# facebookresearch/theseus

Hardware: AMD Instinct MI355X
Metric: LM iterations/sec (batch x vars) on SE3 pose-graph (higher is better)
Workload: dtype f32

## Files before the change

include/theseus_hip.h:

```cpp
#ifndef THESEUS_HIP_H_
#define THESEUS_HIP_H_

#include <stdint.h>

#ifdef __cplusplus
extern "C" {
#endif

#define THX_F32 0
#define THX_F64 1
#define THX_TILE 128

typedef struct {
  double near_zero;
  double d_near_zero;
  double near_pi;
} thx_lie_eps;

typedef struct {
  int32_t num_poses;
  int32_t num_edges;
  int32_t num_priors;
  const int32_t* edge_i;
  const int32_t* edge_j;
// ... 121 lines not shown
  const int32_t* th_mask32;
  const int32_t* th_k0h;
  const int32_t* rg0_rows;
  const int32_t* rg0_zf;
  const int32_t* rg0_tile_ptr;
  const int32_t* rg0_piece_blk;
  const int32_t* rg0_piece_rc;
  int32_t rg0_ngroups;
  int32_t rg0_max_tile_pieces;
  const int32_t* sc_pair_host;
  const int32_t* sc_perm;
  const int32_t* sc_mask;
  const int32_t* row_first;
} thx_hblock_layout;
int thx_hblock_fill_mask(int32_t nvars, int32_t bd, int32_t nblocks, const int32_t* blocks, int32_t* mask);
int thx_pg_assemble_blocks(const thx_pg_structure* s, const thx_pg_data* d, const thx_hblock_layout* layout, void* Hc,
                           int64_t bstride, void* g, int dtype, const thx_lie_eps* eps, void* stream);
int thx_hblocks_expand(const thx_hblock_layout* layout, const void* Hc, int64_t bstride, int32_t B, void* H, int64_t ld,
                       int dtype, void* stream);
int thx_hblocks_diag(const thx_hblock_layout* layout, const void* Hc, int64_t bstride, int32_t B, void* d, int64_t ldv,
                     int dtype, void* stream);

typedef struct {
  int32_t row0, col0, dof_a, dof_b, term_begin, term_end, elem_begin, pad_;
} thx_block_target;
typedef struct {
  const void* Ja;
  const void* Jb;
  int64_t bstride_a, bstride_b;
  int32_t dim, dof_a, dof_b, pad_;
// ... 309 lines not shown
```

theseus_amd/_lib.py:

```python
import ctypes
import os
from ctypes import POINTER, Structure, c_char_p, c_double, c_int, c_int32, c_int64, c_void_p

import torch

_HERE = os.path.dirname(os.path.abspath(__file__))
LIB_PATH = os.environ.get("THESEUS_HIP_LIB") or os.path.join(_HERE, "lib", "libtheseus_hip.so")

THX_TILE = 128
THX_ERR_CHUNKS = 128
THX_LU_MAX_N = 4096
THX_BA_ERR_CHUNKS = 256
TRAJ2_COLLISION, TRAJ2_GP, TRAJ2_PRIOR = 0, 1, 2
PUSH2_QSP, PUSH2_MFB, PUSH2_CONTACT, PUSH2_PRIOR = 0, 1, 2, 3
HOMOG_ALIGN, HOMOG_PRIOR = 0, 1
THX_HOMOG_CHUNK = 1024
THX_HOMOG_SUMS = 10
LOSS_NONE, LOSS_WELSCH, LOSS_HUBER, LOSS_HINGE = 0, 1, 2, 3
LOSS_FLATTEN = 4
LOSS_GEMAN_MCCLURE = 8
ABI_VERSION = 30


class LieEps(Structure):
# ... 59 lines not shown
        (k, c_void_p) for k in ("rg_group_ptr_host", "rg_rows", "rg_k0", "rg_tile_ptr", "rg_piece_blk", "rg_piece_rc")] + [
        ("rg_max_tile_pieces", c_int32)] + [
        (k, c_void_p) for k in ("rg_zf", "tr_tile_host", "tr_perm16", "tr_mask16", "th_tile_host", "th_perm32", "th_mask32", "th_k0h",
                                "rg0_rows", "rg0_zf", "rg0_tile_ptr", "rg0_piece_blk", "rg0_piece_rc")] + [
        ("rg0_ngroups", c_int32), ("rg0_max_tile_pieces", c_int32)] + [
        (k, c_void_p) for k in ("sc_pair_host", "sc_perm", "sc_mask", "row_first")]


def hblock_fill_mask(blocks, nvars: int, bd: int):
    import numpy as np
    b = np.ascontiguousarray(np.asarray(blocks, dtype=np.int32).reshape(-1, 2))
    ntiles = (nvars * bd + THX_TILE - 1) // THX_TILE
    mask = np.zeros((ntiles, 4 * ntiles), dtype=np.int32)
    check(load().thx_hblock_fill_mask(nvars, bd, b.shape[0], b.ctypes.data, mask.ctypes.data), "thx_hblock_fill_mask")
    return mask


def max_offdiag_tile_pieces(tile_ptr, ntiles: int) -> int:
    import numpy as np
    cnt = np.diff(np.asarray(tile_ptr, dtype=np.int64))
    if cnt.size < ntiles * (ntiles + 1) // 2 or ntiles < 2:
        return 0
    off = np.ones(ntiles * (ntiles + 1) // 2, bool)
    i = np.arange(ntiles)
    off[i * (i + 1) // 2 + i] = False
    return int(cnt[: off.size][off].max())


class SE2Eps(Structure):
    _fields_ = [("near_zero", c_double), ("d_near_zero", c_double)]
# ... 92 lines not shown
                        c_void_p, c_int, c_void_p, POINTER(CholSchedule)],
    "thx_chol_factor_forward": [c_void_p, c_int64, c_int32, c_int32, c_void_p, c_int, c_double, c_void_p, c_void_p,
                                c_void_p, c_void_p, c_void_p, c_int64, c_int, c_void_p, POINTER(CholSchedule)],
    "thx_chol_factor_sparse": [c_void_p, c_int64, c_int32, c_int32, c_void_p, c_int, c_double, c_void_p, c_void_p, c_void_p,
                               c_void_p, c_void_p, c_int64, POINTER(TilePattern), c_int, c_void_p, POINTER(CholSchedule)],
    "thx_chol_solve_sparse": [c_void_p, c_int64, c_int32, c_int32, c_void_p, c_void_p, c_void_p, c_int64, c_int,
                              POINTER(TilePattern), c_int, c_void_p],
    "thx_pg_assemble_blocks": [POINTER(PGStructure), POINTER(PGData), POINTER(HBlockLayout), c_void_p, c_int64, c_void_p, c_int,
                               POINTER(LieEps), c_void_p],
    "thx_hblocks_expand": [POINTER(HBlockLayout), c_void_p, c_int64, c_int32, c_void_p, c_int64, c_int, c_void_p],
    "thx_hblocks_diag": [POINTER(HBlockLayout), c_void_p, c_int64, c_int32, c_void_p, c_int64, c_int, c_void_p],
    "thx_chol_factor_hblocks": [POINTER(HBlockLayout), c_void_p, c_int64, c_int32, c_int32, c_void_p, c_int, c_double, c_void_p,
                                c_int64, c_void_p, c_void_p, c_void_p, c_void_p, c_int64, POINTER(TilePattern), c_int, c_void_p,
                                POINTER(CholSchedule)],
    "thx_hblock_fill_mask": [c_int32, c_int32, c_int32, c_void_p, c_void_p],
    "thx_chol_plan": [c_int32, c_int64, c_int32, c_int, c_int, c_int, c_int64, POINTER(HBlockLayout), POINTER(CholSchedule),
                      POINTER(CholPlanInfo)],
    "thx_chol_factor_levels": [POINTER(HBlockLayout), c_void_p, c_int64, c_int32, c_void_p, c_int, c_double, c_void_p, c_void_p,
                               c_void_p, c_void_p, c_void_p, c_int64, POINTER(TilePattern), POINTER(LevelSchedule), c_int, c_void_p,
                               POINTER(CholSchedule)],
    "thx_chol_solve_levels": [c_void_p, c_int32, c_void_p, c_void_p, c_void_p, c_int64, c_int, POINTER(TilePattern),
                              POINTER(LevelSchedule), c_int, c_void_p],
    "thx_vec_gather": [c_void_p, c_int64, c_void_p, c_int64, c_void_p, c_int32, c_int32, c_int, c_void_p],
    "thx_chol_solve": [c_void_p, c_int64, c_int32, c_int32, c_void_p, c_void_p, c_void_p, c_int64, c_int,
                       c_void_p],
    "thx_chol_solve_backward": [c_void_p, c_int64, c_int32, c_int32, c_void_p, c_void_p, c_void_p, c_int64, c_int,
                                c_void_p],
    "thx_chol_solve_env": [c_void_p, c_int64, c_int32, c_int32, c_void_p, c_void_p, c_void_p, c_int64, c_void_p, c_int,
                           c_void_p],
    "thx_chol_solve_backward_env": [c_void_p, c_int64, c_int32, c_int32, c_void_p, c_void_p, c_void_p, c_int64, c_void_p, c_int,
# ... 96 lines not shown
```

theseus_amd/build.py:

```python
import os
import re
import subprocess
import sys

HERE = os.path.dirname(os.path.abspath(__file__))
CSRC = os.path.join(HERE, "csrc")
LIBDIR = os.path.join(HERE, "lib")
LIB = os.path.join(LIBDIR, "libtheseus_hip.so")
SOURCES = ["pg_kernels.hip", "chol_kernels.hip", "pg_vjp_kernels.hip", "block_kernels.hip", "pg2_kernels.hip", "ba_kernels.hip", "pgso3_kernels.hip", "pgso2_kernels.hip", "ba_vjp_kernels.hip", "vjp_unroll_ba_kernels.hip", "lu_kernels.hip", "multi_solve_kernels.hip", "traj_kernels.hip", "push_kernels.hip", "homog_kernels.hip"]
FLAGS = ["--offload-arch=gfx950", "-O3", "-std=c++17", "-fPIC", "-Wno-unused-value", "-Wno-pass-failed"]


def _mtime(p):
    return os.path.getmtime(p) if os.path.exists(p) else 0.0


def deps(path):
    seen, todo = set(), [os.path.normpath(path)]
    while todo:
        f = todo.pop()
        if f in seen:
            continue
        seen.add(f)
        with open(f) as fh:
# ... 30 lines not shown
```

theseus_amd/compiler.py:

```python
from dataclasses import dataclass, field
from typing import List, Optional, Sequence, Tuple

import numpy as np
import torch

from . import _lib

DOF = 6


@dataclass
class PoseGraphStructure:

    num_poses: int
    edge_i: np.ndarray
    edge_j: np.ndarray
    prior_pose: np.ndarray
    edge_row_start: np.ndarray = None
    prior_row_start: np.ndarray = None
    inc_ptr: np.ndarray = field(default=None, repr=False)
    inc_edge: np.ndarray = field(default=None, repr=False)
    inc_side: np.ndarray = field(default=None, repr=False)
    inc_other: np.ndarray = field(default=None, repr=False)
    pri_ptr: np.ndarray = field(default=None, repr=False)
# ... 520 lines not shown
                self.t["sc_" + f] = torch.from_numpy(np.ascontiguousarray(getattr(pc, f))).to(device)
                setattr(c, "sc_" + f, self.t["sc_" + f].data_ptr())
        tr = hb.tile_rows()
        if tr is not None:
            self.tr_tile_host = np.ascontiguousarray(tr.has)
            c.tr_tile_host = self.tr_tile_host.ctypes.data
            for f in ("perm", "mask"):
                self.t["tr_" + f + "16"] = torch.from_numpy(np.ascontiguousarray(getattr(tr, f))).to(device)
                setattr(c, "tr_" + f + "16", self.t["tr_" + f + "16"].data_ptr())
            self.th_tile_host = np.ascontiguousarray(tr.has32)
            c.th_tile_host = self.th_tile_host.ctypes.data
            for f in ("perm32", "mask32", "k0h"):
                self.t["th_" + f] = torch.from_numpy(np.ascontiguousarray(getattr(tr, f))).to(device)
                setattr(c, "th_" + f, self.t["th_" + f].data_ptr())
        self.c = c
```

theseus_amd/kernels.py:

```python
import ctypes
import dataclasses
from dataclasses import dataclass
from typing import Callable, Optional

import torch

from . import _lib
from .compiler import DeviceStructure

_LIE_EPS = {
    torch.float32: dict(near_zero=1e-2, d_near_zero=2e-1, near_pi=1e-2),
    torch.float64: dict(near_zero=5e-3, d_near_zero=1e-2, near_pi=1e-7),
}
_SE2_EPS = {
    torch.float32: dict(near_zero=3e-2, d_near_zero=1e-1),
    torch.float64: dict(near_zero=1e-6, d_near_zero=1e-3),
}
_FLAGS = dict(fast_approx_local_jacobians=False)
_REFERENCE_PARAMS = None


def use_reference_global_params(theseus_params) -> None:
    global _REFERENCE_PARAMS
    _REFERENCE_PARAMS = theseus_params
# ... 375 lines not shown
    def pg_assemble_blocks(self, s: DeviceStructure, t: PGTensors, hb, Hc, g, poses=None):
        if t.group != "SE3":
            raise RuntimeError("the block-compact Hessian is implemented for SE3 pose graphs")
        dt = Hc.dtype
        _lib.check(self.lib.thx_pg_assemble_blocks(s.c, t.c_struct(poses), hb.c, _lib.ptr(Hc, "Hc"), Hc.stride(0), _lib.ptr(g, "g"),
                                                   _lib.dtype_code(dt), lie_eps(dt), _lib.stream_ptr(Hc.device)),
                   "thx_pg_assemble_blocks")

    def hblocks_expand(self, hb, Hc, H):
        _lib.check(self.lib.thx_hblocks_expand(hb.c, _lib.ptr(Hc), Hc.stride(0), Hc.shape[0], _lib.ptr(H), H.shape[-1],
                                               _lib.dtype_code(Hc.dtype), _lib.stream_ptr(Hc.device)), "thx_hblocks_expand")

    def hblocks_diag(self, hb, Hc, d):
        _lib.check(self.lib.thx_hblocks_diag(hb.c, _lib.ptr(Hc), Hc.stride(0), Hc.shape[0], _lib.ptr(d), d.stride(0),
                                             _lib.dtype_code(Hc.dtype), _lib.stream_ptr(Hc.device)), "thx_hblocks_diag")

    def chol_factor_hblocks(self, hb, Hc, n, damping, ellipsoidal, damping_eps, L, panels, info, pattern=None, rhs=None, y=None):
        B, ld = L.shape[0], (0 if L.dim() == 4 else L.shape[-1])
        _lib.check(self.lib.thx_chol_factor_hblocks(
            hb.c, _lib.ptr(Hc), Hc.stride(0), n, B, _lib.ptr(damping), int(bool(ellipsoidal)), float(damping_eps), _lib.ptr(L), ld,
            _lib.ptr(panels), _lib.ptr(info), _lib.ptr(rhs), _lib.ptr(y), rhs.stride(0) if rhs is not None else n,
            pattern.c_struct(L.device) if pattern is not None else None, _lib.dtype_code(L.dtype), _lib.stream_ptr(L.device),
            self._sched()), "thx_chol_factor_hblocks")

    def chol_factor_levels(self, layout, Hc, damping, ellipsoidal, damping_eps, L, panels, info, pattern, rhs=None, y=None):
        dev = L.device
        _lib.check(self.lib.thx_chol_factor_levels(
            layout.c, _lib.ptr(Hc), Hc.stride(0), L.shape[0], _lib.ptr(damping), int(bool(ellipsoidal)), float(damping_eps),
            _lib.ptr(L), _lib.ptr(panels), _lib.ptr(info), _lib.ptr(rhs), _lib.ptr(y), y.stride(0) if y is not None else 0,
            pattern.c_struct(dev), pattern.c_levels(dev), _lib.dtype_code(L.dtype), _lib.stream_ptr(dev), self._sched()),
# ... 410 lines not shown
```

theseus_amd/linear_solver.py:

```python
import abc
import math
import warnings
from typing import Any, Dict, Optional, Sequence, Type, Union

import torch

from .core import Objective
from .linearization import HipLinearization, Linearization
from . import _lib


class LinearSolver(abc.ABC):
    def __init__(self, objective: Objective, linearization_cls: Optional[Type[Linearization]] = None,
                 linearization_kwargs: Optional[Dict[str, Any]] = None, **kwargs):
        linearization_kwargs = linearization_kwargs or {}
        self.linearization: Linearization = linearization_cls(objective, **linearization_kwargs)

    def reset(self, **kwargs):
        pass

    @abc.abstractmethod
    def solve(self, damping: Optional[Union[float, torch.Tensor]] = None, **kwargs) -> torch.Tensor:
        pass


class HipCholeskyCore:

    def _core_init(self):
        self.K = self.linearization.K
        self.L = self.panels = self.info = self._y = None
        self._lam = None
        self.factor_version = 0

    def _ensure_buffers(self):
        lin = self.linearization
        g = lin.g
        shape = (g.shape[0], lin.ld, lin.ld)
        if self.L is None or tuple(self.L.shape) != shape or self.L.device != g.device or self.L.dtype != g.dtype:
            B = g.shape[0]
            nt = (lin.n + _lib.THX_TILE - 1) // _lib.THX_TILE
            self.L = torch.zeros(shape, dtype=g.dtype, device=g.device)
            self.panels = torch.empty(B, nt, _lib.THX_TILE, _lib.THX_TILE, dtype=g.dtype, device=g.device)
            self._y = torch.empty(B, lin.n, dtype=g.dtype, device=g.device)
            self.info = torch.zeros(B, dtype=torch.int32, device=g.device)
            self._lam = torch.empty(B, dtype=g.dtype, device=g.device)
            self._unfused_forward = False

    def _linearized(self) -> bool:
        lin = self.linearization
        return lin.linearized if hasattr(lin, "linearized") else lin.H is not None

    def _factor_call(self, lam, ellipsoidal_damping, damping_eps, rhs, y, pattern=None):
        lin = self.linearization
        if getattr(lin, "_compact", False):
            self.K.chol_factor_hblocks(lin.hblocks, lin.Hc, lin.n, lam, ellipsoidal_damping, damping_eps, self.L, self.panels,
                                       self.info, pattern=pattern, rhs=rhs, y=y)
        elif pattern is not None:
            self.K.chol_factor_sparse(lin.H, lin.n, lam, ellipsoidal_damping, damping_eps, self.L, self.panels, self.info,
                                      pattern, rhs=rhs, y=y)
        else:
            self.K.chol_factor(lin.H, lin.n, lam, ellipsoidal_damping, damping_eps, self.L, self.panels, self.info, rhs=rhs, y=y)

    def factorize(self, damping: Optional[Union[float, torch.Tensor]] = None, ellipsoidal_damping: bool = True,
                  damping_eps: float = 1e-8, rhs: Optional[torch.Tensor] = None):
        if not self._linearized():
            raise RuntimeError("linearize() must be called before solve().")
        self._ensure_buffers()
        lam = None
        if damping is not None:
            lam = self._lam
            if isinstance(damping, torch.Tensor):
                lam.copy_(damping.to(lam.dtype).expand(lam.shape[0]))
            else:
                lam.fill_(float(damping))
        y = self._y if rhs is not None else None
        self.factor_version += 1
        self._factored_with = (lam is not None, bool(ellipsoidal_damping), float(damping_eps))
        self._factor_call(lam, ellipsoidal_damping, damping_eps, rhs, y)
        return y

    def solve_with_factor(self, rhs: torch.Tensor) -> torch.Tensor:
        rhs = rhs.contiguous()
        x = torch.empty_like(rhs)
        self._substitute(rhs, x, backward_only=False)
        return x

    def factor_snapshot(self):
        return self.L.clone(), self.panels.clone()

    def solve_with_snapshot(self, snapshot, rhs: torch.Tensor) -> torch.Tensor:
        L, panels = snapshot
        rhs = rhs.contiguous()
        x = torch.empty_like(rhs)
        self.K.chol_solve(L, self.linearization.n, panels, rhs, x, **self._envelope())
        return x

    solve_envelope = True

    def _envelope(self) -> Dict[str, torch.Tensor]:
        lin = self.linearization
        if self.solve_envelope and getattr(lin, "_compact", False) and lin.hblocks is not None:
            return {"row_first": lin.hblocks.t["row_first"]}
        return {}

    def _substitute(self, rhs, x, backward_only: bool):
        if backward_only:
            self.K.chol_solve_backward(self.L, self.linearization.n, self.panels, rhs, x, **self._envelope())
        else:
            self.K.chol_solve(self.L, self.linearization.n, self.panels, rhs, x, **self._envelope())

    def _factor_owner(self) -> "HipCholeskyCore":
        return self

    def _factorize_undamped(self) -> "HipCholeskyCore":
        self.factorize(None)
        self.check_info()
        return self

    def solve_multi_with_factor(self, rhs: torch.Tensor, which: int = 0) -> torch.Tensor:
        own = self._factor_owner()
        if own is None or own.L is None or own.factor_version == 0:
            raise RuntimeError("solve_multi_with_factor: nothing has been factorised yet (solve() or factorize() first).")
        n = own.linearization.n
        if rhs.dim() != 3 or rhs.shape[0] != own.L.shape[0] or rhs.shape[2] != n or rhs.shape[1] < 1:
            raise ValueError(f"solve_multi_with_factor: rhs must be (B = {own.L.shape[0]}, k >= 1, n = {n}), got {tuple(rhs.shape)}")
        x = rhs.detach().to(own.L.dtype).clone(memory_format=torch.contiguous_format)
        own.K.chol_solve_multi(own.L, n, own.panels, x, x, which=which)
        return x

    @torch.no_grad()
    def sample_deltas(self, n_samples: int = 10, temperature: float = 1.0, noise: Optional[torch.Tensor] = None,
                      generator: Optional[torch.Generator] = None) -> torch.Tensor:
        if not temperature > 0:
            raise ValueError(f"sample_deltas: temperature must be positive, got {temperature}")
        if int(n_samples) < 1:
            raise ValueError(f"sample_deltas: n_samples must be at least 1, got {n_samples}")
        delta = self.solve()
        own = self._factor_owner()
        B, n = delta.shape
        if noise is None:
            noise = torch.randn(n, int(n_samples), generator=generator, device=delta.device, dtype=delta.dtype)
        if noise.dim() == 2 and tuple(noise.shape) == (n, n_samples):
            y = noise.t().unsqueeze(0).expand(B, n_samples, n)
        elif noise.dim() == 3 and tuple(noise.shape) == (B, n, n_samples):
            y = noise.transpose(1, 2)
        else:
            raise ValueError(f"sample_deltas: noise must be ({n}, {n_samples}) or ({B}, {n}, {n_samples}), got {tuple(noise.shape)}")
        y = y.to(device=delta.device, dtype=delta.dtype).clone(memory_format=torch.contiguous_format)
        own.K.chol_solve_multi(own.L, n, own.panels, y, y, which=1)
        y.mul_(math.sqrt(float(temperature))).add_(delta.unsqueeze(1))
        return y.transpose(1, 2)

    @torch.no_grad()
    def marginal_covariance(self, var_names: Sequence[str]) -> torch.Tensor:
        lin = self.linearization
        names = list(var_names)
        if len(set(names)) != len(names):
            raise ValueError(f"marginal_covariance: repeated variable names in {names}")
        cols = []
        for name in names:
            try:
                k = lin.ordering.index_of(name)
            except KeyError:
                raise ValueError(f"marginal_covariance: {name!r} is not an optimisation variable of the objective") from None
            cols.extend(range(lin.var_start_cols[k], lin.var_start_cols[k] + lin.var_dims[k]))
        if not cols:
            raise ValueError("marginal_covariance: no variables named")
        own = self._factorize_undamped()
        B, n, d = own.L.shape[0], own.linearization.n, len(cols)
        idx = torch.tensor(cols, dtype=torch.long, device=own.L.device)
        E = torch.zeros(B, d, n, dtype=own.L.dtype, device=own.L.device)
        E[:, torch.arange(d, device=idx.device), idx] = 1
        own.K.chol_solve_multi(own.L, n, own.panels, E, E, which=0)
        C = E[:, :, idx]
        return (C + C.transpose(1, 2)) / 2

    def check_info(self):
        bad = self.info.nonzero()
        if bad.numel():
            b = int(bad[0])
            raise RuntimeError(
                f"linalg.cholesky: (Batch element {b}): The factorization could not be completed because the "
                f"input is not positive-definite (the leading minor of order {int(self.info[b])} is not "
                "positive-definite).")

    def singular_mask(self) -> torch.Tensor:
        return (self.linearization.diagonal() == 0).any(dim=1)

# ... 28 lines not shown
            singular = self.singular_mask()
            self._last_singular = singular
            delta.masked_fill_(singular.unsqueeze(1), 0.0)
            self.info.masked_fill_(singular, 0)
            seen = singular.any()
            self._singular_seen = seen if getattr(self, "_singular_seen", None) is None else (self._singular_seen | seen)
            if check_info:
                self.post_singular_warning()
        if check_info:
            self.check_info()
        return delta


class HipCholeskySolver(HipCholeskyCore, LinearSolver):
    def __init__(self, objective: Objective, linearization_cls: Optional[Type[Linearization]] = None,
                 linearization_kwargs: Optional[Dict[str, Any]] = None, check_singular: bool = False, **kwargs):
        linearization_cls = linearization_cls or HipLinearization
        if not (isinstance(linearization_cls, type) and issubclass(linearization_cls, HipLinearization)):
            raise RuntimeError("HipCholeskySolver only works with theseus_amd.HipLinearization, "
                               f"but {linearization_cls} was provided.")
        LinearSolver.__init__(self, objective, linearization_cls, linearization_kwargs)
        self._check_singular = check_singular
        self._core_init()

    def solve(self, damping: Optional[Union[float, torch.Tensor]] = None, ellipsoidal_damping: bool = True,
              damping_eps: float = 1e-8, check_info: bool = True, **kwargs) -> torch.Tensor:
        return self._solve(damping, ellipsoidal_damping, damping_eps, check_info)


def _dense_cholesky_only(name: str):
    def method(self, *args, **kwargs):
# ... 62 lines not shown
    def _substitute(self, rhs, x, backward_only: bool):
        if backward_only:
            self.K.lu_solve_backward(self.LU, self.linearization.n, rhs, x)
        else:
            self.K.lu_solve(self.LU, self.linearization.n, self.piv, rhs, x)

    def check_info(self):
        bad = self.info.nonzero()
        if bad.numel():
            b = int(bad[0])
            raise RuntimeError(f"linalg.solve: (Batch element {b}): The solver failed because the input matrix is singular.")


class HipLUSolver(HipLUCore, LinearSolver):
    def __init__(self, objective: Objective, linearization_cls: Optional[Type[Linearization]] = None,
                 linearization_kwargs: Optional[Dict[str, Any]] = None, check_singular: bool = False, **kwargs):
        linearization_cls = linearization_cls or HipLinearization
        if not (isinstance(linearization_cls, type) and issubclass(linearization_cls, HipLinearization)):
            raise RuntimeError("HipLUSolver only works with theseus_amd.HipLinearization, "
                               f"but {linearization_cls} was provided.")
        LinearSolver.__init__(self, objective, linearization_cls, linearization_kwargs)
        self._check_singular = check_singular
        self._core_init()

    def solve(self, damping: Optional[Union[float, torch.Tensor]] = None, ellipsoidal_damping: bool = True,
              damping_eps: float = 1e-8, check_info: bool = True, **kwargs) -> torch.Tensor:
        return self._solve(damping, ellipsoidal_damping, damping_eps, check_info)
```

theseus_amd/plugin.py:

```python
from typing import Any, Dict, List, Optional, Type, Union

import torch

import theseus as th
from theseus.optimizer import Linearization as _RefLinearization
from theseus.optimizer.linear import CholeskyDenseSolver as _RefCholeskyDenseSolver
from theseus.optimizer.linear import LUDenseSolver as _RefLUDenseSolver
from theseus.optimizer.linear import LinearSolver as _RefLinearSolver

from theseus.global_params import _THESEUS_GLOBAL_PARAMS as _REF_GLOBAL_PARAMS

from .generic import BlockAssembler
from .autograd import detached_tensors, pg_vjp_grads
from .kernels import default_kernels, round_up
from .linear_solver import HipCholeskyCore, HipLUCore
from .linearization import HipLinearizationCore
from .packed import UnsupportedObjective
from . import kernels as _kernels

_kernels.use_reference_global_params(_REF_GLOBAL_PARAMS)


def _refuse_unrolled_av(lin):
    if getattr(lin, "_unroll", None) is not None and torch.is_grad_enabled():
# ... 470 lines not shown
        self.K.diag(self.H, self.n, d)
        return d


class _TensorSystemSolver(HipCholeskyCore):
    def __init__(self, K, check_singular: bool):
        self.linearization = _TensorSystem(K)
        self._check_singular = check_singular
        self._core_init()


class HipCholeskySolver(HipCholeskyCore, _RefCholeskyDenseSolver):

    def __init__(self, objective: th.Objective, linearization_cls: Optional[Type[_RefLinearization]] = None,
                 linearization_kwargs: Optional[Dict[str, Any]] = None, check_singular: bool = False,
                 lagged_failure_check: bool = False, **kwargs):
        linearization_cls = linearization_cls or HipLinearization
        if not (isinstance(linearization_cls, type) and issubclass(linearization_cls, HipLinearization)):
            raise RuntimeError("HipCholeskySolver only works with theseus_amd.plugin.HipLinearization, "
                               f"but {linearization_cls} was provided.")
        _RefLinearSolver.__init__(self, objective, linearization_cls, linearization_kwargs)
        self._check_singular = check_singular
        self._core_init()
        self._lagged = bool(lagged_failure_check)
        self._lag = None

    def reset(self, **kwargs):
        if self._lagged and self._lag is not None and self._lag.seen():
            self._lag = None
            import warnings
            warnings.warn("HipCholeskySolver(lagged_failure_check=True): the last linear solve of the previous optimize() failed "
# ... 303 lines not shown
```

Before: 107,900.

## Add fill-reducing variable reordering for sparse Cholesky of compact Hessian blocks

Adds a host-side reordering pass (Cuthill-McKee and King orderings scored by envelope size) that permutes pose variables to shrink the envelope of the block Hessian. The compact Hessian blocks are permuted on device into the new order, factored there, and the right-hand side and solution are gathered into and out of the permuted frame. It aims to cut the fill and work of the envelope/tiled Cholesky factor and solve. It adds permute and gather kernels each iteration plus a one-time ordering cost, and it is only used when the ordering beats the natural order.

Result: faster. 131,200 (median of 6 runs) (+21.6%).

```diff
diff --git a/include/theseus_hip.h b/include/theseus_hip.h
--- a/include/theseus_hip.h
+++ b/include/theseus_hip.h
@@ -159,6 +159,11 @@
   const int32_t* row_first;
 } thx_hblock_layout;
 int thx_hblock_fill_mask(int32_t nvars, int32_t bd, int32_t nblocks, const int32_t* blocks, int32_t* mask);
+int thx_hblock_order(int32_t nvars, int32_t bd, int32_t nblocks, const int32_t* blocks, int32_t* perm_out, int64_t* score_out);
+int thx_hblocks_permute(const void* src, int64_t sstride, void* dst, int64_t dstride, const int32_t* map, int32_t nblocks, int32_t bd,
+                        int32_t B, int dtype, void* stream);
+int thx_frame_permute(const void* H, int64_t ld, void* Hp, int64_t ldp, const int32_t* idx, int32_t n, int32_t B, int dtype,
+                      void* stream);
 int thx_pg_assemble_blocks(const thx_pg_structure* s, const thx_pg_data* d, const thx_hblock_layout* layout, void* Hc,
                            int64_t bstride, void* g, int dtype, const thx_lie_eps* eps, void* stream);
 int thx_hblocks_expand(const thx_hblock_layout* layout, const void* Hc, int64_t bstride, int32_t B, void* H, int64_t ld,
diff --git a/theseus_amd/_lib.py b/theseus_amd/_lib.py
--- a/theseus_amd/_lib.py
+++ b/theseus_amd/_lib.py
@@ -97,6 +97,15 @@
     mask = np.zeros((ntiles, 4 * ntiles), dtype=np.int32)
     check(load().thx_hblock_fill_mask(nvars, bd, b.shape[0], b.ctypes.data, mask.ctypes.data), "thx_hblock_fill_mask")
     return mask
+
+
+def hblock_order(blocks, nvars: int, bd: int):
+    import numpy as np
+    b = np.ascontiguousarray(np.asarray(blocks, dtype=np.int32).reshape(-1, 2))
+    perm = np.zeros(nvars, dtype=np.int32)
+    score = np.zeros(2, dtype=np.int64)
+    check(load().thx_hblock_order(nvars, bd, b.shape[0], b.ctypes.data, perm.ctypes.data, score.ctypes.data), "thx_hblock_order")
+    return perm, int(score[0]), int(score[1])
 
 
 def max_offdiag_tile_pieces(tile_ptr, ntiles: int) -> int:
@@ -219,6 +228,9 @@
                                 c_int64, c_void_p, c_void_p, c_void_p, c_void_p, c_int64, POINTER(TilePattern), c_int, c_void_p,
                                 POINTER(CholSchedule)],
     "thx_hblock_fill_mask": [c_int32, c_int32, c_int32, c_void_p, c_void_p],
+    "thx_hblock_order": [c_int32, c_int32, c_int32, c_void_p, c_void_p, c_void_p],
+    "thx_hblocks_permute": [c_void_p, c_int64, c_void_p, c_int64, c_void_p, c_int32, c_int32, c_int32, c_int, c_void_p],
+    "thx_frame_permute": [c_void_p, c_int64, c_void_p, c_int64, c_void_p, c_int32, c_int32, c_int, c_void_p],
     "thx_chol_plan": [c_int32, c_int64, c_int32, c_int, c_int, c_int, c_int64, POINTER(HBlockLayout), POINTER(CholSchedule),
                       POINTER(CholPlanInfo)],
     "thx_chol_factor_levels": [POINTER(HBlockLayout), c_void_p, c_int64, c_int32, c_void_p, c_int, c_double, c_void_p, c_void_p,
diff --git a/theseus_amd/build.py b/theseus_amd/build.py
--- a/theseus_amd/build.py
+++ b/theseus_amd/build.py
@@ -7,7 +7,7 @@
 CSRC = os.path.join(HERE, "csrc")
 LIBDIR = os.path.join(HERE, "lib")
 LIB = os.path.join(LIBDIR, "libtheseus_hip.so")
-SOURCES = ["pg_kernels.hip", "chol_kernels.hip", "pg_vjp_kernels.hip", "block_kernels.hip", "pg2_kernels.hip", "ba_kernels.hip", "pgso3_kernels.hip", "pgso2_kernels.hip", "ba_vjp_kernels.hip", "vjp_unroll_ba_kernels.hip", "lu_kernels.hip", "multi_solve_kernels.hip", "traj_kernels.hip", "push_kernels.hip", "homog_kernels.hip"]
+SOURCES = ["pg_kernels.hip", "chol_kernels.hip", "hblock_order.hip", "pg_vjp_kernels.hip", "block_kernels.hip", "pg2_kernels.hip", "ba_kernels.hip", "pgso3_kernels.hip", "pgso2_kernels.hip", "ba_vjp_kernels.hip", "vjp_unroll_ba_kernels.hip", "lu_kernels.hip", "multi_solve_kernels.hip", "traj_kernels.hip", "push_kernels.hip", "homog_kernels.hip"]
 FLAGS = ["--offload-arch=gfx950", "-O3", "-std=c++17", "-fPIC", "-Wno-unused-value", "-Wno-pass-failed"]
 
 
diff --git a/theseus_amd/compiler.py b/theseus_amd/compiler.py
--- a/theseus_amd/compiler.py
+++ b/theseus_amd/compiler.py
@@ -558,3 +558,53 @@
                 self.t["th_" + f] = torch.from_numpy(np.ascontiguousarray(getattr(tr, f))).to(device)
                 setattr(c, "th_" + f, self.t["th_" + f].data_ptr())
         self.c = c
+
+
+class _OrderedPattern:
+
+    def __init__(self, dof: int, nvars: int, pattern: np.ndarray):
+        self.dof, self.num_poses, self._pattern = dof, nvars, pattern
+        self.inc_ptr = np.zeros(nvars + 1, dtype=np.int32)
+        self.inc_other = np.zeros(0, dtype=np.int32)
+
+    def lower_block_pattern(self) -> np.ndarray:
+        return self._pattern
+
+
+class OrderedHessianBlocks:
+
+    def __init__(self, hb: HessianBlocks, perm: np.ndarray):
+        d, P = hb.bd, hb.nvars
+        perm = np.asarray(perm, dtype=np.int64)
+        if perm.shape != (P,) or not np.array_equal(np.sort(perm), np.arange(P)):
+            raise ValueError("OrderedHessianBlocks: perm is not a permutation of the layout's variables")
+        pos = np.empty(P, dtype=np.int64)
+        pos[perm] = np.arange(P)
+        a, b = pos[hb.blocks[:, 0]], pos[hb.blocks[:, 1]]
+        swapped = a < b
+        pat = np.stack([np.maximum(a, b), np.minimum(a, b)], axis=1)
+        self.base, self.perm, self.pos = hb, perm.astype(np.int32), pos.astype(np.int32)
+        self.layout = HessianBlocks(_OrderedPattern(d, P, pat[np.lexsort((pat[:, 1], pat[:, 0]))]))
+        ident = {(int(p), int(q)): k for k, (p, q) in enumerate(self.layout.blocks.tolist())}
+        self.block_map = np.zeros(hb.nblocks, dtype=np.int32)
+        for k, ((p, q), t) in enumerate(zip(pat.tolist(), swapped.tolist())):
+            self.block_map[ident[(p, q)]] = (k << 1) | int(t)
+        self.nswapped = int(swapped.sum())
+        self.to_perm = (d * perm[:, None] + np.arange(d)[None, :]).reshape(-1).astype(np.int32)
+        self.from_perm = (d * pos[:, None] + np.arange(d)[None, :]).reshape(-1).astype(np.int32)
+        self._dev = {}
+
+    def on(self, device):
+        key = str(device)
+        if key not in self._dev:
+            maps = {f: torch.from_numpy(getattr(self, f)).to(device) for f in ("block_map", "to_perm", "from_perm")}
+            self._dev[key] = (self.layout.on(device), maps)
+        return self._dev[key]
+
+
+def ordered_hessian_blocks(hb: HessianBlocks) -> Optional[OrderedHessianBlocks]:
+    cached = getattr(hb, "_ordered", None)
+    if cached is None:
+        perm, score, natural = _lib.hblock_order(hb.blocks, hb.nvars, hb.bd)
+        cached = hb._ordered = OrderedHessianBlocks(hb, perm) if score < natural else False
+    return cached or None
diff --git a/theseus_amd/csrc/hblock_order.hip b/theseus_amd/csrc/hblock_order.hip
--- /dev/null
+++ b/theseus_amd/csrc/hblock_order.hip
@@ -0,0 +1,280 @@
+#include <algorithm>
+#include <cstdint>
+#include <vector>
+
+#include "common.cuh"
+
+namespace thx {
+namespace {
+
+struct VarGraph {
+  int32_t n = 0;
+  std::vector<int32_t> ptr, adj;
+  int32_t deg(int32_t v) const { return ptr[v + 1] - ptr[v]; }
+};
+
+bool build_graph(int32_t nvars, int32_t nblocks, const int32_t* blocks, VarGraph& g) {
+  std::vector<std::pair<int32_t, int32_t>> e;
+  e.reserve(2 * (size_t)nblocks);
+  for (int32_t k = 0; k < nblocks; ++k) {
+    const int32_t p = blocks[2 * k], q = blocks[2 * k + 1];
+    if (p < 0 || p >= nvars || q < 0 || q > p) return false;
+    if (q < p) {
+      e.emplace_back(p, q);
+      e.emplace_back(q, p);
+    }
+  }
+  std::sort(e.begin(), e.end());
+  e.erase(std::unique(e.begin(), e.end()), e.end());
+  g.n = nvars;
+  g.ptr.assign(nvars + 1, 0);
+  g.adj.resize(e.size());
+  for (auto& x : e) ++g.ptr[x.first + 1];
+  for (int32_t v = 0; v < nvars; ++v) g.ptr[v + 1] += g.ptr[v];
+  for (size_t k = 0; k < e.size(); ++k) g.adj[k] = e[k].second;
+  return true;
+}
+
+int64_t envelope_score(const VarGraph& g, int32_t bd, const std::vector<int32_t>& order, std::vector<int32_t>& pos) {
+  for (int32_t k = 0; k < g.n; ++k) pos[order[k]] = k;
+  int64_t s = 0;
+  for (int32_t k = 0; k < g.n; ++k) {
+    const int32_t v = order[k];
+    int32_t f = k;
+    for (int32_t a = g.ptr[v]; a < g.ptr[v + 1]; ++a) f = std::min(f, pos[g.adj[a]]);
+    const int64_t w = (int64_t)bd * (k - f);
+    for (int32_t i = 0; i < bd; ++i) s += (w + i) * (w + i);
+  }
+  return s;
+}
+
+std::pair<int32_t, int32_t> bfs_far(const VarGraph& g, int32_t s, std::vector<int32_t>& level, std::vector<int32_t>& queue) {
+  std::fill(level.begin(), level.end(), -1);
+  queue.clear();
+  queue.push_back(s);
+  level[s] = 0;
+  for (size_t h = 0; h < queue.size(); ++h) {
+    const int32_t v = queue[h];
+    for (int32_t a = g.ptr[v]; a < g.ptr[v + 1]; ++a)
+      if (level[g.adj[a]] < 0) {
+        level[g.adj[a]] = level[v] + 1;
+        queue.push_back(g.adj[a]);
+      }
+  }
+  const int32_t last = level[queue.back()];
+  int32_t best = queue.back();
+  for (int32_t v : queue)
+    if (level[v] == last && (g.deg(v) < g.deg(best) || (g.deg(v) == g.deg(best) && v < best))) best = v;
+  return {best, last + 1};
+}
+
+std::pair<int32_t, int32_t> pseudo_peripheral(const VarGraph& g, int32_t s, std::vector<int32_t>& level, std::vector<int32_t>& queue) {
+  int32_t u = s;
+  auto fu = bfs_far(g, u, level, queue);
+  for (int it = 0; it < 8; ++it) {
+    const int32_t v = fu.first;
+    const auto fv = bfs_far(g, v, level, queue);
+    if (fv.second <= fu.second) return {u, v};
+    u = v;
+    fu = fv;
+  }
+  return {u, fu.first};
+}
+
+void cuthill_mckee(const VarGraph& g, int32_t start, std::vector<int32_t>& order) {
+  std::vector<char> seen(g.n, 0);
+  std::vector<int32_t> nb;
+  order.clear();
+  int32_t next_free = 0;
+  for (int32_t s = start; (int32_t)order.size() < g.n;) {
+    size_t h = order.size();
+    order.push_back(s);
+    seen[s] = 1;
+    for (; h < order.size(); ++h) {
+      const int32_t v = order[h];
+      nb.clear();
+      for (int32_t a = g.ptr[v]; a < g.ptr[v + 1]; ++a)
+        if (!seen[g.adj[a]]) nb.push_back(g.adj[a]);
+      std::sort(nb.begin(), nb.end(), [&](int32_t x, int32_t y) { return g.deg(x) != g.deg(y) ? g.deg(x) < g.deg(y) : x < y; });
+      for (int32_t w : nb) {
+        seen[w] = 1;
+        order.push_back(w);
+      }
+    }
+    while (next_free < g.n && seen[next_free]) ++next_free;
+    s = next_free;
+  }
+}
+
+void king(const VarGraph& g, int32_t start, std::vector<int32_t>& order) {
+  constexpr int32_t NUMBERED = -2, OUT = -1;
+  std::vector<int32_t> since(g.n, OUT);
+  std::vector<int32_t> front;
+  order.clear();
+  int32_t pick = start;
+  for (int32_t step = 0; step < g.n; ++step) {
+    if (pick < 0) {
+      int64_t bestg = INT64_MAX;
+      for (int32_t v : front) {
+        int32_t grow = 0;
+        for (int32_t a = g.ptr[v]; a < g.ptr[v + 1]; ++a) grow += since[g.adj[a]] == OUT;
+        const int64_t key = ((int64_t)grow << 32) | since[v];
+        if (key < bestg || (key == bestg && v < pick)) {
+          bestg = key;
+          pick = v;
+        }
+      }
+      if (pick < 0)
+        for (int32_t v = 0; v < g.n; ++v)
+          if (since[v] == OUT && (pick < 0 || g.deg(v) < g.deg(pick))) pick = v;
+    }
+    if (since[pick] >= 0) front.erase(std::find(front.begin(), front.end(), pick));
+    since[pick] = NUMBERED;
+    order.push_back(pick);
+    for (int32_t a = g.ptr[pick]; a < g.ptr[pick + 1]; ++a)
+      if (since[g.adj[a]] == OUT) {
+        since[g.adj[a]] = step;
+        front.push_back(g.adj[a]);
+      }
+    pick = -1;
+  }
+}
+
+}
+
+template <typename T>
+__global__ void hblocks_permute_kernel(const T* __restrict__ src, int64_t sstride, T* __restrict__ dst, int64_t dstride,
+                                       const int32_t* __restrict__ map, int nelems, int bd) {
+  const int b = blockIdx.y, idx = blockIdx.x * blockDim.x + threadIdx.x;
+  if (idx >= nelems) return;
+  const int bb = bd * bd, k = idx / bb, e = idx % bb;
+  const int m = map[k];
+  const int se = (m & 1) ? (e % bd) * bd + e / bd : e;
+  dst[(int64_t)b * dstride + idx] = src[(int64_t)b * sstride + (int64_t)(m >> 1) * bb + se];
+}
+
+template <typename T>
+__global__ void hblocks_permute4_kernel(const T* __restrict__ src, int64_t sstride, T* __restrict__ dst, int64_t dstride,
+                                        const int32_t* __restrict__ map, int nquads, int bd) {
+  typedef T T4 __attribute__((ext_vector_type(4)));
+  const int b = blockIdx.y, q = blockIdx.x * blockDim.x + threadIdx.x;
+  if (q >= nquads) return;
+  const int bb = bd * bd, qb = bb / 4, k = q / qb, e0 = 4 * (q % qb);
+  const int m = map[k];
+  const T* from = src + (int64_t)b * sstride + (int64_t)(m >> 1) * bb;
+  T4 v;
+  if (m & 1) {
+#pragma unroll
+    for (int i = 0; i < 4; ++i) v[i] = from[((e0 + i) % bd) * bd + (e0 + i) / bd];
+  } else {
+    v = *reinterpret_cast<const T4*>(from + e0);
+  }
+  *reinterpret_cast<T4*>(dst + (int64_t)b * dstride + (int64_t)k * bb + e0) = v;
+}
+
+template <typename T>
+__global__ void frame_permute_kernel(const T* __restrict__ H, int64_t ld, T* __restrict__ Hp, int64_t ldp,
+                                     const int32_t* __restrict__ idx, int n) {
+  const int b = blockIdx.z, i = blockIdx.y, j = blockIdx.x * blockDim.x + threadIdx.x;
+  if (j > i) return;
+  const int a = idx[i], c = idx[j];
+  Hp[(int64_t)b * ldp * ldp + (int64_t)i * ldp + j] = H[(int64_t)b * ld * ld + (int64_t)max(a, c) * ld + min(a, c)];
+}
+
+}
+
+using namespace thx;
+
+int thx_hblock_order(int32_t nvars, int32_t bd, int32_t nblocks, const int32_t* blocks, int32_t* perm_out, int64_t* score_out) {
+  if (nvars <= 0 || bd <= 0 || nblocks < 0 || (nblocks > 0 && !blocks) || !perm_out) return fail("thx_hblock_order: bad arguments");
+  if ((int64_t)nvars * bd > (int64_t)1 << 20) return fail("thx_hblock_order: matrix too large");
+  VarGraph g;
+  if (!build_graph(nvars, nblocks, blocks, g)) return fail("thx_hblock_order: a block outside tril(H)");
+  std::vector<int32_t> best(nvars), cand, rev, pos(nvars), level(nvars), queue;
+  for (int32_t v = 0; v < nvars; ++v) best[v] = v;
+  const int64_t natural = envelope_score(g, bd, best, pos);
+  int64_t best_score = natural;
+  auto offer = [&](const std::vector<int32_t>& o) {
+    const int64_t s = envelope_score(g, bd, o, pos);
+    if (s < best_score) {
+      best_score = s;
+      best = o;
+    }
+  };
+  auto offer_both = [&](const std::vector<int32_t>& o) {
+    offer(o);
+    rev.assign(o.rbegin(), o.rend());
+    offer(rev);
+  };
+  std::vector<int32_t> starts;
+  const auto ends = pseudo_peripheral(g, 0, level, queue);
+  starts = {ends.first, ends.second, 0, nvars - 1};
+  {
+    std::vector<int32_t> by_deg(nvars);
+    for (int32_t v = 0; v < nvars; ++v) by_deg[v] = v;
+    const int32_t take = std::min<int32_t>(4, nvars);
+    std::partial_sort(by_deg.begin(), by_deg.begin() + take, by_deg.end(),
+                      [&](int32_t x, int32_t y) { return g.deg(x) != g.deg(y) ? g.deg(x) < g.deg(y) : x < y; });
+    starts.insert(starts.end(), by_deg.begin(), by_deg.begin() + take);
+  }
+  {
+    std::vector<int32_t> uniq;
+    for (int32_t s : starts)
+      if (std::find(uniq.begin(), uniq.end(), s) == uniq.end()) uniq.push_back(s);
+    starts.swap(uniq);
+  }
+  cuthill_mckee(g, ends.first, cand);
+  offer_both(cand);
+  cuthill_mckee(g, ends.second, cand);
+  offer_both(cand);
+  if (nvars <= 16384)
+    for (int32_t s : starts) {
+      king(g, s, cand);
+      offer_both(cand);
+    }
+  std::copy(best.begin(), best.end(), perm_out);
+  if (score_out) {
+    score_out[0] = best_score;
+    score_out[1] = natural;
+  }
+  return 0;
+}
+
+int thx_hblocks_permute(const void* src, int64_t sstride, void* dst, int64_t dstride, const int32_t* map, int32_t nblocks, int32_t bd,
+                        int32_t B, int dtype, void* stream) {
+  if (!src || !dst || !map || nblocks <= 0 || bd <= 0 || B <= 0 || B > 65535 || src == dst) return fail("thx_hblocks_permute: bad args");
+  const int64_t nelems = (int64_t)nblocks * bd * bd;
+  if (nelems > INT32_MAX || sstride < nelems || dstride < nelems) return fail("thx_hblocks_permute: the lists are shorter than nblocks blocks");
+  const size_t vec = dtype == THX_F64 ? 32 : 16;
+  if ((bd * bd) % 4 == 0 && sstride % 4 == 0 && dstride % 4 == 0 && reinterpret_cast<uintptr_t>(src) % vec == 0 &&
+      reinterpret_cast<uintptr_t>(dst) % vec == 0) {
+    const int nquads = (int)(nelems / 4);
+    dim3 grid4((unsigned)((nquads + 255) / 256), B);
+    THX_DISPATCH(dtype,
+                 hipLaunchKernelGGL(hblocks_permute4_kernel<float>, grid4, dim3(256), 0, as_stream(stream), (const float*)src, sstride,
+                                    (float*)dst, dstride, map, nquads, bd),
+                 hipLaunchKernelGGL(hblocks_permute4_kernel<double>, grid4, dim3(256), 0, as_stream(stream), (const double*)src,
+                                    sstride, (double*)dst, dstride, map, nquads, bd));
+    return check_launch("thx_hblocks_permute");
+  }
+  dim3 grid((unsigned)((nelems + 255) / 256), B), block(256);
+  THX_DISPATCH(dtype,
+               hipLaunchKernelGGL(hblocks_permute_kernel<float>, grid, block, 0, as_stream(stream), (const float*)src, sstride,
+                                  (float*)dst, dstride, map, (int)nelems, bd),
+               hipLaunchKernelGGL(hblocks_permute_kernel<double>, grid, block, 0, as_stream(stream), (const double*)src, sstride,
+                                  (double*)dst, dstride, map, (int)nelems, bd));
+  return check_launch("thx_hblocks_permute");
+}
+
+int thx_frame_permute(const void* H, int64_t ld, void* Hp, int64_t ldp, const int32_t* idx, int32_t n, int32_t B, int dtype,
+                      void* stream) {
+  if (!H || !Hp || !idx || n <= 0 || n > 65535 || B <= 0 || B > 65535 || ld < n || ldp < n || H == Hp)
+    return fail("thx_frame_permute: bad args");
+  dim3 grid((n + 255) / 256, n, B), block(256);
+  THX_DISPATCH(dtype,
+               hipLaunchKernelGGL(frame_permute_kernel<float>, grid, block, 0, as_stream(stream), (const float*)H, ld, (float*)Hp,
+                                  ldp, idx, n),
+               hipLaunchKernelGGL(frame_permute_kernel<double>, grid, block, 0, as_stream(stream), (const double*)H, ld,
+                                  (double*)Hp, ldp, idx, n));
+  return check_launch("thx_frame_permute");
+}
diff --git a/theseus_amd/kernels.py b/theseus_amd/kernels.py
--- a/theseus_amd/kernels.py
+++ b/theseus_amd/kernels.py
@@ -413,6 +413,20 @@
     def hblocks_diag(self, hb, Hc, d):
         _lib.check(self.lib.thx_hblocks_diag(hb.c, _lib.ptr(Hc), Hc.stride(0), Hc.shape[0], _lib.ptr(d), d.stride(0),
                                              _lib.dtype_code(Hc.dtype), _lib.stream_ptr(Hc.device)), "thx_hblocks_diag")
+
+    def hblocks_permute(self, src, dst, block_map, bd):
+        if src.dim() != 2 or dst.dim() != 2 or src.shape[0] != dst.shape[0] or src.dtype != dst.dtype or block_map.dtype != torch.int32:
+            raise ValueError(f"hblocks_permute: src {tuple(src.shape)} {src.dtype} / dst {tuple(dst.shape)} {dst.dtype} / map "
+                             f"{block_map.dtype} do not fit")
+        _lib.check(self.lib.thx_hblocks_permute(_lib.ptr(src), src.stride(0), _lib.ptr(dst), dst.stride(0), _lib.ptr(block_map),
+                                                block_map.numel(), bd, src.shape[0], _lib.dtype_code(src.dtype),
+                                                _lib.stream_ptr(src.device)), "thx_hblocks_permute")
+
+    def frame_permute(self, H, Hp, idx, n):
+        if H.dim() != 3 or Hp.dim() != 3 or H.shape[0] != Hp.shape[0] or H.dtype != Hp.dtype or idx.dtype != torch.int32 or idx.numel() < n:
+            raise ValueError(f"frame_permute: H {tuple(H.shape)} {H.dtype} / Hp {tuple(Hp.shape)} {Hp.dtype} / idx {idx.dtype} do not fit")
+        _lib.check(self.lib.thx_frame_permute(_lib.ptr(H), H.shape[-1], _lib.ptr(Hp), Hp.shape[-1], _lib.ptr(idx), n, H.shape[0],
+                                              _lib.dtype_code(H.dtype), _lib.stream_ptr(H.device)), "thx_frame_permute")
 
     def chol_factor_hblocks(self, hb, Hc, n, damping, ellipsoidal, damping_eps, L, panels, info, pattern=None, rhs=None, y=None):
         B, ld = L.shape[0], (0 if L.dim() == 4 else L.shape[-1])
diff --git a/theseus_amd/linear_solver.py b/theseus_amd/linear_solver.py
--- a/theseus_amd/linear_solver.py
+++ b/theseus_amd/linear_solver.py
@@ -24,23 +24,81 @@
         pass
 
 
+class _FactorSnapshot(tuple):
+    ordered = None
+
+
 class HipCholeskyCore:
+
+    ordering = "auto"
 
     def _core_init(self):
         self.K = self.linearization.K
-        self.L = self.panels = self.info = self._y = None
+        self._L = self._panels = self.info = self._y = None
         self._lam = None
         self.factor_version = 0
+        self._factor_ord = None
+        self._Hp = self._gp = self._xp = None
+        self._natural_frame = None
+        self._force_natural = False
+
+    @property
+    def L(self):
+        return self._L if self._factor_ord is None else self._natural_factor()[0]
+
+    @L.setter
+    def L(self, value):
+        self._L = value
+
+    @property
+    def panels(self):
+        return self._panels if self._factor_ord is None else self._natural_factor()[1]
+
+    @panels.setter
+    def panels(self, value):
+        self._panels = value
+
+    def _natural_factor(self):
+        if self._natural_frame is None or self._natural_frame[0] != self.factor_version:
+            lin = self.linearization
+            L, panels = torch.zeros_like(self._L), torch.empty_like(self._panels)
+            has_lam, ellipsoidal, eps = self._factored_with
+            if getattr(lin, "_compact", False):
+                self.K.chol_factor_hblocks(lin.hblocks, lin.Hc, lin.n, self._lam if has_lam else None, ellipsoidal, eps, L, panels,
+                                           torch.zeros_like(self.info))
+            else:
+                self.K.chol_factor(lin.H, lin.n, self._lam if has_lam else None, ellipsoidal, eps, L, panels, torch.zeros_like(self.info))
+            self._natural_frame = (self.factor_version, L, panels)
+        return self._natural_frame[1:]
+
+    def _ordered(self):
+        lin = self.linearization
+        if self.ordering == "natural" or self._force_natural:
+            return None
+        if self.ordering != "auto":
+            raise ValueError(f"ordering must be 'auto' or 'natural', got {self.ordering!r}")
+        packed = getattr(lin, "packed", None)
+        if getattr(lin, "_compact", False) and lin.hblocks is not None:
+            host, dev = lin.hblocks.host, lin.Hc.device
+        elif (not getattr(lin, "_compact", False) and getattr(packed, "supports_block_hessian", lambda: False)()
+              and getattr(lin, "full_matrix", None) is None and lin.H is not None):
+            host, dev = packed.structure.hessian_blocks(), lin.H.device
+        else:
+            return None
+        from .compiler import ordered_hessian_blocks
+        oh = ordered_hessian_blocks(host)
+        return None if oh is None else oh.on(dev)
 
     def _ensure_buffers(self):
         lin = self.linearization
         g = lin.g
         shape = (g.shape[0], lin.ld, lin.ld)
-        if self.L is None or tuple(self.L.shape) != shape or self.L.device != g.device or self.L.dtype != g.dtype:
+        if self._L is None or tuple(self._L.shape) != shape or self._L.device != g.device or self._L.dtype != g.dtype:
             B = g.shape[0]
             nt = (lin.n + _lib.THX_TILE - 1) // _lib.THX_TILE
-            self.L = torch.zeros(shape, dtype=g.dtype, device=g.device)
-            self.panels = torch.empty(B, nt, _lib.THX_TILE, _lib.THX_TILE, dtype=g.dtype, device=g.device)
+            self._L = torch.zeros(shape, dtype=g.dtype, device=g.device)
+            self._panels = torch.empty(B, nt, _lib.THX_TILE, _lib.THX_TILE, dtype=g.dtype, device=g.device)
+            self._Hp = self._gp = self._xp = self._natural_frame = None
             self._y = torch.empty(B, lin.n, dtype=g.dtype, device=g.device)
             self.info = torch.zeros(B, dtype=torch.int32, device=g.device)
             self._lam = torch.empty(B, dtype=g.dtype, device=g.device)
@@ -52,14 +110,35 @@
 
     def _factor_call(self, lam, ellipsoidal_damping, damping_eps, rhs, y, pattern=None):
         lin = self.linearization
-        if getattr(lin, "_compact", False):
-            self.K.chol_factor_hblocks(lin.hblocks, lin.Hc, lin.n, lam, ellipsoidal_damping, damping_eps, self.L, self.panels,
+        self._factor_ord = self._natural_frame = None
+        ordered = self._ordered() if pattern is None else None
+        if ordered is not None:
+            layout, maps = ordered
+            compact = getattr(lin, "_compact", False)
+            shape = (lin.Hc.shape[0], layout.host.bstride) if compact else tuple(lin.H.shape)
+            if self._Hp is None or tuple(self._Hp.shape) != shape:
+                self._Hp = torch.zeros(shape, dtype=self._L.dtype, device=self._L.device)
+                self._gp, self._xp = torch.empty_like(self._y), torch.empty_like(self._y)
+            if rhs is not None:
+                self.K.vec_gather(rhs.contiguous(), self._gp, maps["to_perm"])
+            rhs_p = self._gp if rhs is not None else None
+            if compact:
+                self.K.hblocks_permute(lin.Hc, self._Hp, maps["block_map"], layout.host.bd)
+                self.K.chol_factor_hblocks(layout, self._Hp, lin.n, lam, ellipsoidal_damping, damping_eps, self._L, self._panels,
+                                           self.info, rhs=rhs_p, y=y)
+            else:
+                self.K.frame_permute(lin.H, self._Hp, maps["to_perm"], lin.n)
+                self.K.chol_factor(self._Hp, lin.n, lam, ellipsoidal_damping, damping_eps, self._L, self._panels, self.info,
+                                   rhs=rhs_p, y=y)
+            self._factor_ord = ordered
+        elif getattr(lin, "_compact", False):
+            self.K.chol_factor_hblocks(lin.hblocks, lin.Hc, lin.n, lam, ellipsoidal_damping, damping_eps, self._L, self._panels,
                                        self.info, pattern=pattern, rhs=rhs, y=y)
         elif pattern is not None:
-            self.K.chol_factor_sparse(lin.H, lin.n, lam, ellipsoidal_damping, damping_eps, self.L, self.panels, self.info,
+            self.K.chol_factor_sparse(lin.H, lin.n, lam, ellipsoidal_damping, damping_eps, self._L, self._panels, self.info,
                                       pattern, rhs=rhs, y=y)
         else:
-            self.K.chol_factor(lin.H, lin.n, lam, ellipsoidal_damping, damping_eps, self.L, self.panels, self.info, rhs=rhs, y=y)
+            self.K.chol_factor(lin.H, lin.n, lam, ellipsoidal_damping, damping_eps, self._L, self._panels, self.info, rhs=rhs, y=y)
 
     def factorize(self, damping: Optional[Union[float, torch.Tensor]] = None, ellipsoidal_damping: bool = True,
                   damping_eps: float = 1e-8, rhs: Optional[torch.Tensor] = None):
@@ -86,28 +165,42 @@
         return x
 
     def factor_snapshot(self):
-        return self.L.clone(), self.panels.clone()
+        snap = _FactorSnapshot((self._L.clone(), self._panels.clone()))
+        snap.ordered = self._factor_ord
+        return snap
 
     def solve_with_snapshot(self, snapshot, rhs: torch.Tensor) -> torch.Tensor:
         L, panels = snapshot
         rhs = rhs.contiguous()
         x = torch.empty_like(rhs)
-        self.K.chol_solve(L, self.linearization.n, panels, rhs, x, **self._envelope())
+        self._solve_frame(L, panels, getattr(snapshot, "ordered", None), rhs, x, backward_only=False)
         return x
 
     solve_envelope = True
 
-    def _envelope(self) -> Dict[str, torch.Tensor]:
+    def _envelope(self, ordered=None) -> Dict[str, torch.Tensor]:
         lin = self.linearization
         if self.solve_envelope and getattr(lin, "_compact", False) and lin.hblocks is not None:
-            return {"row_first": lin.hblocks.t["row_first"]}
+            return {"row_first": (lin.hblocks if ordered is None else ordered[0]).t["row_first"]}
         return {}
 
+    def _solve_frame(self, L, panels, ordered, rhs, x, backward_only: bool):
+        n = self.linearization.n
+        solve = self.K.chol_solve_backward if backward_only else self.K.chol_solve
+        if ordered is None:
+            solve(L, n, panels, rhs, x, **self._envelope())
+            return
+        maps = ordered[1]
+        if rhs is self._y:
+            src = rhs
+        else:
+            self.K.vec_gather(rhs, self._gp, maps["to_perm"])
+            src = self._gp
+        solve(L, n, panels, src, self._xp, **self._envelope(ordered))
+        self.K.vec_gather(self._xp, x, maps["from_perm"])
+
     def _substitute(self, rhs, x, backward_only: bool):
-        if backward_only:
-            self.K.chol_solve_backward(self.L, self.linearization.n, self.panels, rhs, x, **self._envelope())
-        else:
-            self.K.chol_solve(self.L, self.linearization.n, self.panels, rhs, x, **self._envelope())
+        self._solve_frame(self._L, self._panels, self._factor_ord, rhs, x, backward_only)
 
     def _factor_owner(self) -> "HipCholeskyCore":
         return self
@@ -119,13 +212,19 @@
 
     def solve_multi_with_factor(self, rhs: torch.Tensor, which: int = 0) -> torch.Tensor:
         own = self._factor_owner()
-        if own is None or own.L is None or own.factor_version == 0:
+        if own is None or own._L is None or own.factor_version == 0:
             raise RuntimeError("solve_multi_with_factor: nothing has been factorised yet (solve() or factorize() first).")
         n = own.linearization.n
-        if rhs.dim() != 3 or rhs.shape[0] != own.L.shape[0] or rhs.shape[2] != n or rhs.shape[1] < 1:
-            raise ValueError(f"solve_multi_with_factor: rhs must be (B = {own.L.shape[0]}, k >= 1, n = {n}), got {tuple(rhs.shape)}")
-        x = rhs.detach().to(own.L.dtype).clone(memory_format=torch.contiguous_format)
-        own.K.chol_solve_multi(own.L, n, own.panels, x, x, which=which)
+        if rhs.dim() != 3 or rhs.shape[0] != own._L.shape[0] or rhs.shape[2] != n or rhs.shape[1] < 1:
+            raise ValueError(f"solve_multi_with_factor: rhs must be (B = {own._L.shape[0]}, k >= 1, n = {n}), got {tuple(rhs.shape)}")
+        x = rhs.detach().to(own._L.dtype)
+        maps = own._factor_ord[1] if own._factor_ord is not None else None
+        if maps is not None and which != 1:
+            x = x.index_select(2, maps["to_perm"].long())
+        x = x.clone(memory_format=torch.contiguous_format)
+        own.K.chol_solve_multi(own._L, n, own._panels, x, x, which=which)
+        if maps is not None and which != 2:
+            x = x.index_select(2, maps["from_perm"].long())
         return x
 
     @torch.no_grad()
@@ -135,7 +234,11 @@
             raise ValueError(f"sample_deltas: temperature must be positive, got {temperature}")
         if int(n_samples) < 1:
             raise ValueError(f"sample_deltas: n_samples must be at least 1, got {n_samples}")
-        delta = self.solve()
+        self._force_natural = True
+        try:
+            delta = self.solve()
+        finally:
+            self._force_natural = False
         own = self._factor_owner()
         B, n = delta.shape
         if noise is None:
@@ -147,7 +250,7 @@
         else:
             raise ValueError(f"sample_deltas: noise must be ({n}, {n_samples}) or ({B}, {n}, {n_samples}), got {tuple(noise.shape)}")
         y = y.to(device=delta.device, dtype=delta.dtype).clone(memory_format=torch.contiguous_format)
-        own.K.chol_solve_multi(own.L, n, own.panels, y, y, which=1)
+        own.K.chol_solve_multi(own._L, n, own._panels, y, y, which=1)
         y.mul_(math.sqrt(float(temperature))).add_(delta.unsqueeze(1))
         return y.transpose(1, 2)
 
@@ -167,11 +270,13 @@
         if not cols:
             raise ValueError("marginal_covariance: no variables named")
         own = self._factorize_undamped()
-        B, n, d = own.L.shape[0], own.linearization.n, len(cols)
-        idx = torch.tensor(cols, dtype=torch.long, device=own.L.device)
-        E = torch.zeros(B, d, n, dtype=own.L.dtype, device=own.L.device)
+        B, n, d = own._L.shape[0], own.linearization.n, len(cols)
+        idx = torch.tensor(cols, dtype=torch.long, device=own._L.device)
+        if own._factor_ord is not None:
+            idx = own._factor_ord[1]["from_perm"].long()[idx]
+        E = torch.zeros(B, d, n, dtype=own._L.dtype, device=own._L.device)
         E[:, torch.arange(d, device=idx.device), idx] = 1
-        own.K.chol_solve_multi(own.L, n, own.panels, E, E, which=0)
+        own.K.chol_solve_multi(own._L, n, own._panels, E, E, which=0)
         C = E[:, :, idx]
         return (C + C.transpose(1, 2)) / 2
 
@@ -230,7 +335,11 @@
 
 class HipCholeskySolver(HipCholeskyCore, LinearSolver):
     def __init__(self, objective: Objective, linearization_cls: Optional[Type[Linearization]] = None,
-                 linearization_kwargs: Optional[Dict[str, Any]] = None, check_singular: bool = False, **kwargs):
+                 linearization_kwargs: Optional[Dict[str, Any]] = None, check_singular: bool = False, ordering: str = "auto",
+                 **kwargs):
+        if ordering not in ("auto", "natural"):
+            raise ValueError(f"ordering must be 'auto' or 'natural', got {ordering!r}")
+        self.ordering = ordering
         linearization_cls = linearization_cls or HipLinearization
         if not (isinstance(linearization_cls, type) and issubclass(linearization_cls, HipLinearization)):
             raise RuntimeError("HipCholeskySolver only works with theseus_amd.HipLinearization, "
@@ -323,7 +432,8 @@
 
 class HipLUSolver(HipLUCore, LinearSolver):
     def __init__(self, objective: Objective, linearization_cls: Optional[Type[Linearization]] = None,
-                 linearization_kwargs: Optional[Dict[str, Any]] = None, check_singular: bool = False, **kwargs):
+                 linearization_kwargs: Optional[Dict[str, Any]] = None, check_singular: bool = False, ordering: str = "auto",
+                 **kwargs):
         linearization_cls = linearization_cls or HipLinearization
         if not (isinstance(linearization_cls, type) and issubclass(linearization_cls, HipLinearization)):
             raise RuntimeError("HipLUSolver only works with theseus_amd.HipLinearization, "
diff --git a/theseus_amd/plugin.py b/theseus_amd/plugin.py
--- a/theseus_amd/plugin.py
+++ b/theseus_amd/plugin.py
@@ -508,7 +508,10 @@
 
     def __init__(self, objective: th.Objective, linearization_cls: Optional[Type[_RefLinearization]] = None,
                  linearization_kwargs: Optional[Dict[str, Any]] = None, check_singular: bool = False,
-                 lagged_failure_check: bool = False, **kwargs):
+                 lagged_failure_check: bool = False, ordering: str = "auto", **kwargs):
+        if ordering not in ("auto", "natural"):
+            raise ValueError(f"ordering must be 'auto' or 'natural', got {ordering!r}")
+        self.ordering = ordering
         linearization_cls = linearization_cls or HipLinearization
         if not (isinstance(linearization_cls, type) and issubclass(linearization_cls, HipLinearization)):
             raise RuntimeError("HipCholeskySolver only works with theseus_amd.plugin.HipLinearization, "
```
